# luanfujun/Langevin-MCMC

Measured on AMD Instinct MI355X. Metric: MALA chain-steps/sec, torus scene, higher is better.
Workload: dtype f32

## Files before the change

include/lmc_abi.h:

```cpp
#ifndef LMC_ABI_H
#define LMC_ABI_H

#ifdef __cplusplus
extern "C" {
#endif

typedef struct lmc_ctx lmc_ctx;

typedef struct lmc_scene_desc {
    const char *scene_xml;
    int force_diffuse;
    int max_depth;
    int width, height;
    int seed_offset;
    int device;
    int use_gradient;
} lmc_scene_desc;

const char *lmc_last_error(void);

lmc_ctx *lmc_create(const lmc_scene_desc *desc);
void lmc_destroy(lmc_ctx *ctx);
int lmc_device_count(void);

// ... 35 lines not shown
int lmc_mc_stats(lmc_ctx *ctx, long long *out2);
int lmc_mc_accumulate(lmc_ctx *ctx, int spp, long long stream_begin, long long stream_end);
int lmc_mc_coverage(lmc_ctx *ctx, long long *ranges, int cap);
int lmc_mc_read_fixed(lmc_ctx *ctx, long long *words);
int lmc_mc_overflow(lmc_ctx *ctx, long long *n);
int lmc_group_mc_render(lmc_ctx **ctxs, int n, int spp, long long stream_begin, long long stream_end);
int lmc_group_mc_accumulate(lmc_ctx **ctxs, int n, int spp, long long stream_begin, long long stream_end);
int lmc_mc_save(lmc_ctx *ctx, const char *path);
int lmc_mc_load(lmc_ctx *ctx, const char *path);
long long lmc_mc_file_info(const char *path, char *json, long long cap);
int lmc_mc_layer_info(lmc_ctx *ctx, int *mode, int *n_layers, int *cl, int cap);
int lmc_mc_read_layer(lmc_ctx *ctx, int layer, float *rgb);
int lmc_mc_read_layer_fixed(lmc_ctx *ctx, int layer, long long *words);
int lmc_mc_coverage_probe(const long long *adds, int n_adds, long long total, int *accepted, long long *cov, int cov_cap, int *n_cov, long long *comp, int comp_cap, int *n_comp);
int lmc_mc_chunks_probe(long long begin, long long end, long long n_tiles, long long launch_streams, long long *out, int cap);
int lmc_stats(lmc_ctx *ctx, long long *out8, double *weight_sum);
int lmc_chain_summary(lmc_ctx *ctx, int which, float *out, int stride);
int lmc_relocation_stats(lmc_ctx *ctx, long long *out4);
long long lmc_relocation_skipped(lmc_ctx *ctx);
int lmc_resident_stats(lmc_ctx *ctx, long long *out4, double *kernel_ms);
int lmc_step_timing(lmc_ctx *ctx, double *kernel_ms, long long *launches);
int lmc_kernel_timing(lmc_ctx *ctx, double *out3);
int lmc_kernel_timing_split(lmc_ctx *ctx, double *out4);

int lmc_comm_unique_id(unsigned char *out128);
int lmc_comm_init(lmc_ctx *ctx, int n_ranks, int rank, const unsigned char *id128);
int lmc_film_allreduce(lmc_ctx *ctx);
#define LMC_COMM_MAX_SCALARS 64
int lmc_comm_allreduce_f64(lmc_ctx *ctx, double *vals, int n, int op);
int lmc_comm_barrier(lmc_ctx *ctx);
void *lmc_film_device_ptr(lmc_ctx *ctx, long long *n_floats);

int lmc_grad_batch(int c, int l, int n, const float *primary_soa, const float *scene38, const float *vert_soa, float *loglum, float *grad_soa);

int lmc_hess_batch(int c, int l, int n, const float *primary_soa, const float *scene38, const float *vert_soa, float *loglum, float *grad_soa, float *hess_soa);

int lmc_cache_rows(lmc_ctx *ctx, int dim, float *pss, float *weight, float *extra);
int lmc_cache_probe(lmc_ctx *ctx, int dim, int n, const float *u, int *row, const float *query, const int *cl, float *pdf);

int lmc_trace(lmc_ctx *ctx, int n, const float *rays, int *prim, float *t);
int lmc_occluded(lmc_ctx *ctx, int n, const float *rays, int *occluded);
int lmc_rng_probe(int n_seeds, const unsigned long long *seeds, int mode, int n, float mean, float stddev, unsigned *out);
int lmc_kd_probe(int dim, int npts, const float *pts, int nq, const float *q, float radius_sq, int knn, int *out_n, int *out_idx, float *out_dist);
int lmc_lower_bound_probe(int n, const float *cdf, int nq, const float *u, int *out);
int lmc_layout_probe(int nChains, int words, int mode, int batch, int reps, double *msPerLaunch);
int lmc_lean_plan_probe(int bvh_stack_need, int block_threads, int *stack_words, int *lds_words_per_thread, long long *lds_bytes_per_block);
// ... 66 lines not shown
```

langevin-mcmc_amd/__init__.py:

```python
import ctypes
import os

import numpy as np

_HERE = os.path.dirname(os.path.abspath(__file__))
ROOT = os.path.dirname(_HERE)
LIB_PATH = os.environ.get("LMC_LIB") or os.path.join(_HERE, "liblmc_hip.so")
vp = ctypes.c_void_p
c_ll = ctypes.c_longlong


class SceneDesc(ctypes.Structure):
    _fields_ = [
        ("scene_xml", ctypes.c_char_p),
        ("force_diffuse", ctypes.c_int),
        ("max_depth", ctypes.c_int),
        ("width", ctypes.c_int),
        ("height", ctypes.c_int),
        ("seed_offset", ctypes.c_int),
        ("device", ctypes.c_int),
        ("use_gradient", ctypes.c_int),
    ]


# ... 14 lines not shown
        L.lmc_create.restype = vp
        L.lmc_create.argtypes = [ctypes.POINTER(SceneDesc)]
        L.lmc_destroy.argtypes = [vp]
        L.lmc_info.argtypes = [vp, vp]
        L.lmc_scene_params.argtypes = [vp, vp]
        L.lmc_set_option.argtypes = [vp, ctypes.c_char_p, ctypes.c_double]
        L.lmc_chains_init.argtypes = [vp, c_ll, ctypes.c_int, ctypes.c_int, ctypes.c_int, ctypes.c_int, c_ll, c_ll]
        L.lmc_init_result.argtypes = [vp, vp, vp]
        L.lmc_chains_step.argtypes = [vp, ctypes.c_int]
        L.lmc_sync.argtypes = [vp]
        L.lmc_film_read.argtypes = [vp, vp]
        L.lmc_film_clear.argtypes = [vp]
        L.lmc_stats.argtypes = [vp, vp, vp]
        L.lmc_chain_summary.argtypes = [vp, ctypes.c_int, vp, ctypes.c_int]
        L.lmc_step_timing.argtypes = [vp, vp, vp]
        L.lmc_relocation_stats.argtypes = [vp, vp]
        if hasattr(L, "lmc_resident_stats"):
            L.lmc_resident_stats.argtypes = [vp, vp, vp]
        if hasattr(L, "lmc_relocation_skipped"):
            L.lmc_relocation_skipped.argtypes = [vp]
            L.lmc_relocation_skipped.restype = c_ll
        L.lmc_kernel_timing.argtypes = [vp, vp]
        L.lmc_kernel_timing_split.argtypes = [vp, vp]
        L.lmc_get_option.argtypes = [vp, ctypes.c_char_p, vp]
        L.lmc_output_name.argtypes = [vp]
        L.lmc_output_name.restype = ctypes.c_char_p
        L.lmc_image_read.argtypes = [ctypes.c_char_p, vp, vp, vp]
        L.lmc_image_write_exr.argtypes = [ctypes.c_char_p, vp, ctypes.c_int, ctypes.c_int]
        L.lmc_direct_lighting.argtypes = [vp, ctypes.c_int]
        L.lmc_direct_read.argtypes = [vp, vp]
        L.lmc_path_trace.argtypes = [vp, ctypes.c_int]
        L.lmc_bidir_mc.argtypes = [vp, ctypes.c_int]
        if hasattr(L, "lmc_mc_render"):
            L.lmc_mc_render.argtypes = [vp, ctypes.c_int, c_ll, c_ll]
            L.lmc_mc_read.argtypes = [vp, vp]
            L.lmc_mc_stats.argtypes = [vp, vp]
        if hasattr(L, "lmc_mc_accumulate"):
            L.lmc_mc_accumulate.argtypes = [vp, ctypes.c_int, c_ll, c_ll]
            L.lmc_mc_coverage.argtypes = [vp, vp, ctypes.c_int]
            L.lmc_mc_read_fixed.argtypes = [vp, vp]
            L.lmc_mc_overflow.argtypes = [vp, vp]
            L.lmc_group_mc_render.argtypes = [vp, ctypes.c_int, ctypes.c_int, c_ll, c_ll]
            L.lmc_group_mc_accumulate.argtypes = [vp, ctypes.c_int, ctypes.c_int, c_ll, c_ll]
            L.lmc_mc_save.argtypes = [vp, ctypes.c_char_p]
            L.lmc_mc_load.argtypes = [vp, ctypes.c_char_p]
            L.lmc_mc_file_info.argtypes = [ctypes.c_char_p, ctypes.c_char_p, c_ll]
# ... 367 lines not shown
        if lib().lmc_step_table(self.h, P(out), 1 if clear else 0) != 0:
            raise RuntimeError(_err())
        return out

    def step_timing(self):
        ms = ctypes.c_double()
        n = c_ll()
        if lib().lmc_step_timing(self.h, ctypes.byref(ms), ctypes.byref(n)) != 0:
            raise RuntimeError(_err())
        return ms.value, n.value

    def kernel_timing(self):
        out = (ctypes.c_double * 3)()
        if lib().lmc_kernel_timing(self.h, out) != 0:
            raise RuntimeError(_err())
        return out[0], out[1], int(out[2])

    def kernel_timing_split(self):
        out = (ctypes.c_double * 4)()
        if lib().lmc_kernel_timing_split(self.h, out) != 0:
            raise RuntimeError(_err())
        return {"lean_ms": out[0], "large_ms": out[1], "generic_ms": out[2], "lean_steps": int(out[3])}

    def lean_info(self):
        out = (ctypes.c_int * 16)()
        L = lib()
        L.lmc_lean_info.argtypes = [vp, ctypes.POINTER(ctypes.c_int)]
        if L.lmc_lean_info(self.h, out) != 0:
            raise RuntimeError(_err())
        v = list(out)
        return dict(leaf_hist=v[:8], stack_need=v[8], stack_words=v[9], lds=v[10], glossy=v[11], lightless=v[12], quant=v[13], tight=v[14], block=v[15])

    def trace(self, rays):
        rays = np.ascontiguousarray(rays, np.float32)
        n = len(rays)
        prim = np.zeros(n, np.int32)
        t = np.zeros(n, np.float32)
        if lib().lmc_trace(self.h, n, P(rays), P(prim), P(t)) != 0:
            raise RuntimeError(_err())
        return prim, t

    def occluded(self, rays):
        rays = np.ascontiguousarray(rays, np.float32)
        occ = np.zeros(len(rays), np.int32)
        if lib().lmc_occluded(self.h, len(rays), P(rays), P(occ)) != 0:
            raise RuntimeError(_err())
# ... 381 lines not shown
```

langevin-mcmc_amd/csrc/device/kernels.h:

```cpp
#pragma once
#include <hip/hip_runtime.h>

#include "dchain.h"
#include "dstep_params.h"

namespace lmcd {
struct H2Arrays;
struct MalaPipe;
struct H2Bins;
struct H2MCParam;
}

void LaunchSeedRng(int n, long long firstSeed, uint64_t *state, uint32_t *tab, hipStream_t s);
void LaunchLowerBoundProbe(int n, const float *cdf, int nq, const float *u, int *out, hipStream_t s);
void LaunchRngProbe(int nSeeds, const unsigned long long *seeds, int mode, int n, float mean, float stddev, uint32_t *tabScratch, uint32_t *out, hipStream_t s);
void LaunchPluginGrad(int c, int l, const float *in, float *out, int wantGrad, hipStream_t s);
void LaunchPluginHess(int c, int l, const float *in, float *stage , float *out, hipStream_t s);
void LaunchCacheProbe(const lmcd::DCache *cache, int dim, int n, const float *u, int *row, const float *query, const int *cl, float *pdf, hipStream_t s);
void LaunchTransProbe(int n, int mode, const float *x, const float *y, float *o, hipStream_t s);
void LaunchShadeProbe(const lmcd::DScene &S, int op, bool glossy, int n, const int *ints, const float *in, int *ok, float *out, hipStream_t s);
void LaunchStreamProbe(long long nWords, const float *in, float *out, hipStream_t s);
void LaunchAddInto(float *dst, const float *src, size_t n, hipStream_t s);
void LaunchAddIntoF64(double *dst, const double *src, size_t n, hipStream_t s);
void LaunchAddIntoI64(long long *dst, const long long *src, size_t n, hipStream_t s);
// ... 77 lines not shown
                   const int *listCount, int bvhStackNeed, bool glossy, int gridBlocks, hipStream_t s);
void LaunchMalaFinish(const lmcd::DScene &S, const lmcd::DCache *cache, const lmcd::ChainArrays &A, const lmcd::Film &film, const lmcd::StepParams &P, const lmcd::MalaPipe &M,
                      const int *list, const int *listCount, int gridBlocks, hipStream_t s);
void LaunchMalaGrad(const float *rec, const lmcd::H2Bins &bins, int N, const float *scene38 , float *gout, int gridBlocks, hipStream_t s);
void LaunchHessBatch(int c, int l, int n, const float *primarySoA, const float *scene, const float *vertSoA, float *logLum, float *gradSoA, float *hessSoA,
                     hipStream_t s);
void LaunchBuildLists(const lmcd::ChainArrays &A, const lmcd::NextLists &next, int sortPlain, unsigned leanDims, hipStream_t s);
void LaunchInitLists(int n, int *large, int *counts, hipStream_t s);
void LaunchCachePush(const lmcd::ChainArrays &A, const lmcd::CachePushTargets &T, unsigned long long *tileCounts, int *stageCounts , hipStream_t s);
void LaunchCachePushApply(const float *gathered, size_t stageFloats, int world, const lmcd::PushStageLayout &lay, const lmcd::CachePushTargets &T,
                          int *hostCounts , hipStream_t s);
void LaunchLayoutProbe(int N, int words, int mode, int batch, const float *in, float *out, hipStream_t s);
void LaunchSortByTechnique(const unsigned char *nextKind, const int *in, int *out, const int *count, int *blockHist, int maxEntries, hipStream_t s);
void LaunchInclusiveScan(int *v, int n, int *tileSums, hipStream_t s);
struct RelocBuffers {
    unsigned *placedKey;
    int *tileCount, *tileHist;
    int *members;
    int *sorted;
    int *count;
    float *staging;
    int capacity;
    bool fine;
};
size_t RelocTiles(int N);
size_t RelocRecordWords(int maxDepth);
void LaunchRelocIota(int n, int *v, hipStream_t s);
void LaunchRelocate(const lmcd::ChainArrays &A, int maxDepth, const RelocBuffers &B, bool withoutGaussianOnly, hipStream_t s);
void LaunchRelocPlan(const lmcd::ChainArrays &A, int maxDepth, const RelocBuffers &B, bool withoutGaussianOnly, hipStream_t s);
void LaunchRelocFineKey(const lmcd::ChainArrays &A, const int *leafPosOfTri, int numTris, int mode, unsigned long long *keys, const lmcd::TriData *tris, const lmcd::DMaterial *materials, hipStream_t s);
void LaunchRelocMove(const lmcd::ChainArrays &A, int maxDepth, const RelocBuffers &B, hipStream_t s, int keyMode = 0);
struct RelocSortBuffers {
    unsigned *keys[2];
    int *vals[2];
    int *hist;
    int *scanSums;
};
size_t RelocSortBlocks(int N);
void LaunchRadixSort24(const RelocSortBuffers &W, const int *nPtr, int nMax, int *out, hipStream_t s);
void LaunchRelocFullSort(const lmcd::ChainArrays &A, int maxDepth, const RelocBuffers &B, const RelocSortBuffers &W, hipStream_t s);
void LaunchRelocateFine(const lmcd::ChainArrays &A, int maxDepth, const RelocBuffers &B, const RelocSortBuffers &W, bool withoutGaussianOnly, hipStream_t s);
void LaunchBuildCacheGrid(const float *pts, int n, int dim, int G, int m, const int *coord, int *scratchStart, int *scratchCursor, int *scratchWordCount, int *tileSums,
                          uint2 *words, int *cellStart, unsigned short *idx, hipStream_t s);
size_t CkptRecordWords(int maxDepth, bool sampleCache, bool h2mc);
void LaunchCkptPack(const lmcd::ChainArrays &A, int maxDepth, bool sampleCache, const float *h2Gauss, int first, int n, float *staging, hipStream_t s);
void LaunchCkptUnpack(const lmcd::ChainArrays &A, int maxDepth, bool sampleCache, float *h2Gauss, int first, int n, const float *staging, hipStream_t s);
void LaunchLatchKind(const lmcd::ChainArrays &A, const int *large, const int *generic, const int *lean, const int *counts, unsigned char *kindOf, hipStream_t s);
void LaunchChainRows(const lmcd::ChainArrays &A, int which, const int *ids, int n, const unsigned char *kindOf, float *out, hipStream_t s);
// ... 2 lines not shown
```

langevin-mcmc_amd/csrc/device/relocate.hip:

```cpp
#include "dstep.h"
#include "kernels.h"

namespace lmcd {
namespace {

enum : int { RW_FLAGS = 0, RW_SAMPLEIDX, RW_NUMSAMPLES, RW_ADJREJECT, RW_SPLATCOUNT, RW_CHAINID, RW_SCORESUM, RW_LASTSCORESUM, RW_LASTSCORE, RW_PATHWEIGHT, RW_NEXTKIND, RW_RNG_LO, RW_RNG_HI, RW_KEY, RW_RNG_TICKED, RW_SCALARS = 16 };
constexpr int RW_TAB = RW_SCALARS, RW_HEAD = RW_TAB + 64, RW_VERT = RW_HEAD + DPATH_HEAD_WORDS;

struct RecordLayout {
    int nV, nS;
    LMC_HD int Contrib() const { return RW_VERT + 2 * nV * DVERTEX_WORDS; }
    LMC_HD int Splats() const { return Contrib() + CONTRIB_WORDS; }
    LMC_HD int Vectors() const { return Splats() + nS * SPLAT_WORDS; }
    LMC_HD int Gauss() const { return Vectors() + 7 * MAXPSS; }
    LMC_HD int Words() const { return Gauss() + GAUSS_WORDS; }
};

#ifndef LMC_RELOC_ORDER
#define LMC_RELOC_ORDER 1
#endif
#ifndef LMC_RELOC_TILES
#define LMC_RELOC_TILES 0
#endif
LMC_D int SlotKey(const ChainArrays &A, int i, int tiles) {
// ... 31 lines not shown
constexpr int RELOC_TILE = 1024;
LMC_D int MemberKey(const ChainArrays &A, const unsigned *placedKey, int i, bool withoutGaussianOnly, int tiles) {
    if (i >= A.N || A.stepKind[i] != NEXT_LARGE) return -1;
    const int key = SlotKey(A, i, tiles);
    if ((unsigned)key == placedKey[i]) return -1;
    if (withoutGaussianOnly && (A.flags[i] & F_GAUSS)) return -1;
    return key;
}
__global__ void __launch_bounds__(64) k_reloc_count(ChainArrays A, const unsigned *placedKey, int *tileCount, int *tileHist, bool noGauss, int tiles) {
    __shared__ int h[64];
    h[threadIdx.x] = 0;
    __syncthreads();
    const int base = blockIdx.x * RELOC_TILE + threadIdx.x;
    int total = 0;
    for (int j = 0; j < RELOC_TILE / 64; j++) {
        const int key = MemberKey(A, placedKey, base + 64 * j, noGauss, tiles);
        if (key >= 0) atomicAdd(&h[key], 1), total++;
    }
    __syncthreads();
    tileHist[blockIdx.x * 64 + threadIdx.x] = h[threadIdx.x];
    for (int off = 32; off > 0; off >>= 1) total += __shfl_down(total, off);
    if (threadIdx.x == 0) tileCount[blockIdx.x] = total;
}
__global__ void __launch_bounds__(64) k_reloc_offsets(int nTiles, int *tileCount, int *tileHist, int *count, int capacity) {
    const int key = threadIdx.x;
    int total = 0;
#pragma unroll 8
    for (int t = 0; t < nTiles; t++) total += tileHist[t * 64 + key];
    int incl = total;
    for (int off = 1; off < 64; off <<= 1) {
        const int o = __shfl_up(incl, off);
        if (key >= off) incl += o;
    }
    if (key == 63) {
        if (incl > capacity) count[0] = 0, count[1]++;
        else
            count[0] = incl;
    }
    int run = incl - total;
#pragma unroll 8
    for (int t = 0; t < nTiles; t++) {
        const int c = tileHist[t * 64 + key];
        tileHist[t * 64 + key] = run;
        run += c;
    }
    int carry = 0;
    for (int b = 0; b < nTiles; b += 64) {
        const int t = b + threadIdx.x, v = t < nTiles ? tileCount[t] : 0;
        int in = v;
        for (int off = 1; off < 64; off <<= 1) {
            const int o = __shfl_up(in, off);
            if (key >= off) in += o;
        }
        if (t < nTiles) tileCount[t] = carry + in - v;
        carry += __shfl(in, 63);
    }
}
__global__ void __launch_bounds__(64) k_reloc_assign(ChainArrays A, const unsigned *placedKey, const int *tileStart, const int *groupStart, int *members, int *sorted, bool noGauss, int tiles) {
    __shared__ int cursor[64];
    cursor[threadIdx.x] = groupStart[blockIdx.x * 64 + threadIdx.x];
    __syncthreads();
    const int base = blockIdx.x * RELOC_TILE + threadIdx.x;
    int m0 = tileStart[blockIdx.x];
    for (int j = 0; j < RELOC_TILE / 64; j++) {
        const int key = MemberKey(A, placedKey, base + 64 * j, noGauss, tiles);
        const unsigned long long mask = __ballot(key >= 0);
        const unsigned long long below = (1ull << threadIdx.x) - 1ull;
        if (key >= 0) members[m0 + __popcll(mask & below)] = base + 64 * j;
        unsigned long long todo = mask;
        while (todo) {
            const int k = __shfl(key, __ffsll((long long)todo) - 1);
            const unsigned long long same = __ballot(key == k);
            if (key == k) sorted[cursor[k] + __popcll(same & below)] = m0 + __popcll(mask & below);
            __syncthreads();
            if (threadIdx.x == 0) cursor[k] += __popcll(same);
            __syncthreads();
            todo &= ~same;
        }
        m0 += __popcll(mask);
    }
}

LMC_D float *VectorBase(const ChainArrays &A, int v) {
    float *const b[7] = {A.chV1, A.chV2, A.chCurrNewV2, A.chPropNewV1, A.chPropNewV2, A.chPss, A.chLastPss};
    return b[v];
}
// ... 422 lines not shown
        m0 += __popcll(mask);
    }
}

__global__ void __launch_bounds__(256) k_reloc_iota(int n, int *v) {
    const int i = blockIdx.x * 256 + threadIdx.x;
    if (i < n) v[i] = i;
}

}
}

using namespace lmcd;

static RecordLayout MakeRecordLayout(int maxDepth) {
    RecordLayout R;
    R.nV = std::min(MAXD, std::max(maxDepth, 1));
    R.nS = std::min(MAXCONTRIB, (maxDepth + 1) * (maxDepth + 2) / 2);
    return R;
}
size_t RelocRecordWords(int maxDepth) { return (size_t)MakeRecordLayout(maxDepth).Words(); }
void LaunchRelocIota(int n, int *v, hipStream_t s) { hipLaunchKernelGGL(k_reloc_iota, dim3((n + 255) / 256), dim3(256), 0, s, n, v); }
size_t RelocTiles(int N) { return (size_t)(N + RELOC_TILE - 1) / RELOC_TILE; }

static void LaunchMoveKernels(const ChainArrays &A, const RecordLayout &R, const RelocBuffers &B, int tiles, int moveBlocks, hipStream_t s) {
    static const bool coop = !(getenv("LMC_RELOC_COOP") && atoi(getenv("LMC_RELOC_COOP")) == 0);
    if (coop) {
        hipLaunchKernelGGL(k_reloc_gather_coop, dim3(moveBlocks), dim3(64), 0, s, A, R, B.members, B.count, B.staging, B.capacity, tiles);
        hipLaunchKernelGGL(k_reloc_scatter_coop, dim3(moveBlocks), dim3(64), 0, s, A, R, B.members, B.sorted, B.count, B.staging, B.placedKey, B.capacity);
    } else {
        hipLaunchKernelGGL(k_reloc_gather, dim3(moveBlocks), dim3(64), 0, s, A, R, B.members, B.sorted, B.count, B.staging, B.capacity, tiles);
        hipLaunchKernelGGL(k_reloc_scatter, dim3(moveBlocks), dim3(64), 0, s, A, R, B.members, B.sorted, B.count, B.staging, B.placedKey, B.capacity);
    }
}
void LaunchRelocFineKey(const ChainArrays &A, const int *leafPosOfTri, int numTris, int mode, unsigned long long *keys, const TriData *tris, const DMaterial *materials, hipStream_t s) {
    hipLaunchKernelGGL(k_reloc_finekey, dim3((A.N + 255) / 256), dim3(256), 0, s, A, leafPosOfTri, numTris, mode, keys, tris, materials);
}
void LaunchRelocMove(const ChainArrays &A, int maxDepth, const RelocBuffers &B, hipStream_t s, int keyMode) {
    const RecordLayout R = MakeRecordLayout(maxDepth);
    const int moveBlocks = std::min((A.N + 63) / 64, 65536);
    LaunchMoveKernels(A, R, B, keyMode, moveBlocks, s);
}

size_t RelocSortBlocks(int N) { return (size_t)(N + RS_TILE - 1) / RS_TILE; }
void LaunchRadixSort24(const RelocSortBuffers &W, const int *nPtr, int nMax, int *out, hipStream_t s) {
    const int nBlocks = (int)RelocSortBlocks(nMax);
// ... 7 lines not shown
        hipLaunchKernelGGL(k_rs_scatter, dim3(nBlocks), dim3(64), 0, s, kin[pass], vin[pass], kout[pass], vout[pass], nPtr, nMax, 8 * pass, W.hist, nBlocks);
    }
}
void LaunchRelocFullSort(const ChainArrays &A, int maxDepth, const RelocBuffers &B, const RelocSortBuffers &W, hipStream_t s) {
    const int N = A.N;
    hipLaunchKernelGGL(k_rs_set_count, dim3(1), dim3(64), 0, s, B.count, N);
    hipLaunchKernelGGL(k_rs_key, dim3((N + 255) / 256), dim3(256), 0, s, A, W.keys[0]);
    LaunchRadixSort24(W, B.count, N, B.sorted, s);
    hipLaunchKernelGGL(k_reloc_iota, dim3((N + 255) / 256), dim3(256), 0, s, N, B.members);
    LaunchRelocMove(A, maxDepth, B, s, B.fine ? -1 : 0);
}
void LaunchRelocateFine(const ChainArrays &A, int maxDepth, const RelocBuffers &B, const RelocSortBuffers &W, bool withoutGaussianOnly, hipStream_t s) {
    const RecordLayout R = MakeRecordLayout(maxDepth);
    const int N = A.N, nTiles = (N + RELOC_TILE - 1) / RELOC_TILE;
    hipLaunchKernelGGL(k_relf_count, dim3(nTiles), dim3(64), 0, s, A, B.placedKey, B.tileCount, withoutGaussianOnly);
    hipLaunchKernelGGL(k_relf_offsets, dim3(1), dim3(64), 0, s, nTiles, B.tileCount, B.count, B.capacity);
    hipLaunchKernelGGL(k_relf_assign, dim3(nTiles), dim3(64), 0, s, A, B.placedKey, B.tileCount, B.count, B.members, W.keys[0], withoutGaussianOnly);
    LaunchRadixSort24(W, B.count, B.capacity, B.sorted, s);
    const int moveBlocks = std::min((N + 63) / 64, 4096);
    LaunchMoveKernels(A, R, B, -1, moveBlocks, s);
}

void LaunchRelocPlan(const ChainArrays &A, int maxDepth, const RelocBuffers &B, bool withoutGaussianOnly, hipStream_t s) {
    const int N = A.N, nTiles = (N + RELOC_TILE - 1) / RELOC_TILE;
    const int tiles = (LMC_RELOC_TILES && maxDepth <= 6) ? 8 : 0;
    hipLaunchKernelGGL(k_reloc_count, dim3(nTiles), dim3(64), 0, s, A, B.placedKey, B.tileCount, B.tileHist, withoutGaussianOnly, tiles);
    hipLaunchKernelGGL(k_reloc_offsets, dim3(1), dim3(64), 0, s, nTiles, B.tileCount, B.tileHist, B.count, B.capacity);
    hipLaunchKernelGGL(k_reloc_assign, dim3(nTiles), dim3(64), 0, s, A, B.placedKey, B.tileCount, B.tileHist, B.members, B.sorted, withoutGaussianOnly, tiles);
}
void LaunchRelocate(const ChainArrays &A, int maxDepth, const RelocBuffers &B, bool withoutGaussianOnly, hipStream_t s) {
    const RecordLayout R = MakeRecordLayout(maxDepth);
    const int N = A.N;
    const int tiles = (LMC_RELOC_TILES && maxDepth <= 6) ? 8 : 0;
    LaunchRelocPlan(A, maxDepth, B, withoutGaussianOnly, s);
    const int moveBlocks = std::min((N + 63) / 64, 4096);
    LaunchMoveKernels(A, R, B, tiles, moveBlocks, s);
}
```

langevin-mcmc_amd/csrc/host/context.cpp:

```cpp
#include <hip/hip_runtime.h>
#include <dlfcn.h>

#include <algorithm>
#include <chrono>
#include <condition_variable>
#include <mutex>
#include <cstdio>
#include <cstdlib>
#include <cstring>
#include <exception>
#include <functional>
#include <memory>
#include <stdexcept>
#include <string>
#include <thread>
#include <vector>

#include <rccl/rccl.h>

#include "../../../include/lmc_abi.h"
#include "../device/drng.h"
#include "../device/kernels.h"
#include "../device/upload.h"
#include "../device/dh2coop.h"
// ... 771 lines not shown
    else
        c->chPath.Free(), c->chContrib.Free();
    c->pathWeight.Alloc(N), c->lastScoreSum.Alloc(N), c->lastScore.Alloc(N), c->contribList.Alloc(N * MAXCONTRIB * CONTRIB_WORDS, false);
    c->pushData.Alloc(N * GAUSS_WORDS), c->flags.Alloc(N), c->nextKind.Alloc(N + 4), c->adjacentReject.Alloc(N), c->sampleIdx.Alloc(N), c->numSamples.Alloc(N), c->pushDim.Alloc(N);
    c->counters.Alloc(8), c->weightSum.Alloc(1), c->prof.Alloc(16);
    ChainArrays &A = c->A;
    A.N = (int)N;
    A.rngState = c->rngState.p, A.rngTab = c->rngTab.p, A.rngTicked = c->rngTicked.p, A.curPath = c->curPath.p, A.pathBuf1 = c->pathBuf1.p, A.curContrib = c->curContrib.p, A.scoreSum = c->scoreSum.p;
    A.flags = c->flags.p, A.gaussian = c->gaussian.p, A.gaussian1 = c->gaussian1.p, A.curSplat = c->curSplat.p, A.curSplatCount = c->curSplatCount.p;
    A.chV1 = c->chV1.p, A.chV2 = c->chV2.p, A.chCurrNewV2 = c->chCurrNewV2.p, A.chPropNewV1 = c->chPropNewV1.p, A.chPropNewV2 = c->chPropNewV2.p,
    A.chPss = c->chPss.p, A.chLastPss = c->chLastPss.p;
    A.chPath = sampleCache ? c->chPath.p : nullptr, A.chContrib = sampleCache ? c->chContrib.p : nullptr;
    A.pathWeight = c->pathWeight.p, A.lastScoreSum = c->lastScoreSum.p, A.lastScore = c->lastScore.p;
    A.adjacentReject = c->adjacentReject.p, A.sampleIdx = c->sampleIdx.p, A.numSamples = c->numSamples.p;
    A.contribList = c->contribList.p, A.nextKind = c->nextKind.p, A.pushDim = c->pushDim.p, A.pushData = c->pushData.p;
    A.initPath = c->initPath.p, A.initContrib = c->initContrib.p, A.initScoreSum = c->initScoreSum.p, A.initLsAll = c->initLsAll.p, A.initCLAll = c->initCLAll.p;
    A.counters = c->counters.p, A.weightSum = c->weightSum.p, A.prof = c->prof.p;
    c->relocate = true;
    if (const char *e = getenv("LMC_RELOCATE")) c->relocate = atoi(e) != 0;
    if (sampleCache) c->relocate = false;
    c->relocations = 0;
    if (c->relocate) {
        c->chainId.Alloc(N, false), c->slotOf.Alloc(N, false), c->relocTileCount.Alloc(RelocTiles((int)N) + 1, false), c->relocTileHist.Alloc(RelocTiles((int)N) * 64, false), c->relocMembers.Alloc(N, false);
        c->relocSorted.Alloc(N, false), c->relocCount.Alloc(2), c->relocPlacedKey.Alloc(N, false), c->stepKind.Alloc(N + 4, false);
        c->relocStaging.Alloc(N * RelocRecordWords(c->S.opt.maxDepth), false);
        HIP_CHECK(hipMemsetAsync(c->relocPlacedKey.p, 0xff, N * sizeof(unsigned), s));
        HIP_CHECK(hipMemsetAsync(c->stepKind.p, NEXT_LARGE, N, s));
        LaunchRelocIota((int)N, c->chainId.p, s), LaunchRelocIota((int)N, c->slotOf.p, s);
        c->resortEvery = 32;
        if (const char *e = getenv("LMC_RESORT_EVERY")) c->resortEvery = std::max(0, atoi(e));
        if (c->resortEveryOpt >= 0) c->resortEvery = c->resortEveryOpt;
        c->resortFirst = 4;
        if (const char *e = getenv("LMC_RESORT_FIRST")) c->resortFirst = std::max(0, atoi(e));
        if (c->resortFirstOpt >= 0) c->resortFirst = c->resortFirstOpt;
        if (c->S.opt.h2mc) c->resortEvery = 0;
        c->stepsSinceInit = 0, c->resorts = 0;
        c->relocFine = false;
        if (const char *e = getenv("LMC_RELOC_FINE")) c->relocFine = atoi(e) != 0;
        if (c->resortEvery > 0 || c->relocFine) {
            const size_t nb = RelocSortBlocks((int)N);
            for (int k = 0; k < 2; k++) c->sortKeys[k].Alloc(N, false), c->sortVals[k].Alloc(N, false);
            c->sortHist.Alloc(256 * nb, false), c->sortScanSums.Alloc(256 * nb / 2048 + 2, false);
            c->RS = RelocSortBuffers{{c->sortKeys[0].p, c->sortKeys[1].p}, {c->sortVals[0].p, c->sortVals[1].p}, c->sortHist.p, c->sortScanSums.p};
        }
        c->RB = RelocBuffers{c->relocPlacedKey.p, c->relocTileCount.p, c->relocTileHist.p, c->relocMembers.p, c->relocSorted.p, c->relocCount.p, c->relocStaging.p, (int)N, c->relocFine};
        A.chainId = c->chainId.p, A.slotOf = c->slotOf.p, A.stepKind = c->stepKind.p;
    } else {
        A.chainId = nullptr, A.slotOf = nullptr, A.stepKind = nullptr;
        for (auto *b : {&c->chainId, &c->slotOf, &c->relocTileCount, &c->relocTileHist, &c->relocMembers, &c->relocSorted, &c->relocCount}) b->Free();
        c->relocPlacedKey.Free(), c->stepKind.Free(), c->relocStaging.Free();
    }
    if (!U.fromCheckpoint) {
        LaunchSeedRng((int)N, (long long)chainBegin + c->S.opt.seedOffset, c->rngState.p, c->rngTab.p, s);
        LaunchSetupChains(A, chainBegin, perChain, chainsNeedExtra, s);
    }
    c->stepGrid = (int)std::min<size_t>((N + 255) / 256, 4096);
    c->gradStride = c->stepGrid * 256;
    if (const char *e = getenv("LMC_LEAN_BLOCK")) c->leanBlock = std::max(64, std::min(256, atoi(e) / 64 * 64));
    c->sortPlain = c->S.glossy ? 4 : 0;
    if (const char *e = getenv("LMC_SORT_PLAIN")) c->sortPlain = atoi(e);
    c->gradBuf.Alloc(c->useGradient ? (size_t)c->gradStride * 640 : 1, false);
    size_t maxGridCells = 0;
    for (int d = 0; d <= PSS_MAX_LENGTH; d++) {
        CacheDimHost &cd = c->cacheDims[d];
        cd.ready = false;
        cd.relevant = (d % 2 == 0) && d >= 2 * std::max(c->S.opt.minDepth, 3) && d <= 2 * c->S.opt.maxDepth;
        if (cd.relevant) {
            cd.pss.Alloc((size_t)PSS_MAX_SIZE * d), cd.v1.Alloc((size_t)PSS_MAX_SIZE * d), cd.v2.Alloc((size_t)PSS_MAX_SIZE * d);
            cd.weight.Alloc(PSS_MAX_SIZE);
            if (sampleCache) cd.extra.Alloc((size_t)PSS_MAX_SIZE * CACHE_ROW_EXTRA), cd.distCdf.Alloc(PSS_MAX_SIZE + 1);
            cd.gridG = CacheGridG(d), cd.gridM = std::min(c->gridDims, d);
            size_t cells = 1, nbrs = 1;
// ... 550 lines not shown
            CachePack(c, sL);
            if (c->world == 1 && c->earlyApply) CacheApplyLaunch(c, sL), c->appliedEarly = true;
            else if (c->world > 1 && c->group.size() <= 1 && c->comm && c->earlyApply && RcclEarlyExchange() && c->stageLayout.totalFloats > 0) {
                RcclCheck(GetRccl().AllGather(c->pushStage.p, c->pushGather.p, (size_t)c->stageLayout.totalFloats * sizeof(float), ncclUint8, (ncclComm_t)c->comm, sL),
                          "ncclAllGather(cache pushes, large-step stream)");
                CacheApplyLaunch(c, sL), c->appliedEarly = true;
            }
        }
        if (c->relocate) {
            if (c->relocations == 2 && c->RB.capacity == (int)c->N && c->N >= 65536 && c->resortEvery == 0 && !getenv("LMC_RELOC_STAGING_FULL")) {
                static std::mutex stagingMutex;
                std::lock_guard<std::mutex> lock(stagingMutex);
                HIP_CHECK(hipStreamSynchronize(sL));
                const size_t cap = c->N / 2;
                c->RB.staging = nullptr, c->RB.capacity = 0;
                c->relocStaging.Alloc(cap * RelocRecordWords(c->S.opt.maxDepth), false);
                c->RB.staging = c->relocStaging.p, c->RB.capacity = (int)cap;
            }
            if (c->relocFine) LaunchRelocateFine(c->A, c->S.opt.maxDepth, c->RB, c->RS, c->S.opt.h2mc != 0, sL);
            else
                LaunchRelocate(c->A, c->S.opt.maxDepth, c->RB, c->S.opt.h2mc != 0, sL);
            c->relocations++;
        }
    };
    if (!genericFirst) large();
    if (c->timing) HIP_CHECK(hipEventRecord(ev.e[6], sG));
    LaunchGeneric(c, film, P, cur, cnt, next, sG);
    if (c->timing) HIP_CHECK(hipEventRecord(ev.e[7], sG));
    if (genericFirst) large();
    if (c->timing) HIP_CHECK(hipEventRecord(ev.e[1], s));
    if (!c->S.opt.h2mc) LaunchStepSmallPlain(c->S, c->cacheDev.p, c->A, film, P, c->lists[cur][2].p, cnt + 2, next, c->bvhDepth, c->S.glossy != 0, c->leanLdsStack, c->leanBlock, c->profileLean, s);
    if (c->timing) HIP_CHECK(hipEventRecord(ev.e[2], s));
    if (c->overlap) {
        HIP_CHECK(hipEventRecord(c->joinEvent[0], sL));
        HIP_CHECK(hipStreamWaitEvent(s, c->joinEvent[0], 0));
        if (c->needGeneric) {
            HIP_CHECK(hipEventRecord(c->joinEvent[1], sG));
            HIP_CHECK(hipStreamWaitEvent(s, c->joinEvent[1], 0));
        }
    }
    return exchange;
}
void DebugResort(lmc_ctx *c) {
    hipStream_t s = c->stream;
    const int mode = c->pendingResort;
    c->pendingResort = 0;
// ... 231 lines not shown
int lmc_group_chains_step(lmc_ctx **ctxs, int n, int nSteps) {
    LMC_TRY
    std::vector<lmc_ctx *> g(ctxs, ctxs + n);
    for (lmc_ctx *c : g)
        if (c->group != g) throw std::runtime_error("lmc_group_chains_step: not the group lmc_group_chains_init set up");
    RunSteps(g, nSteps);
    return 0;
    LMC_CATCH(-1)
}

int lmc_sync(lmc_ctx *c) {
    LMC_TRY
    HIP_CHECK(hipSetDevice(c->device));
    HIP_CHECK(hipStreamSynchronize(c->stream));
    return 0;
    LMC_CATCH(-1)
}

int lmc_step_timing(lmc_ctx *c, double *kernelMs, long long *launches) {
    LMC_TRY
    HIP_CHECK(hipStreamSynchronize(c->stream));
    double ms = 0;
    c->smallMs = c->largeMs = c->largeOnlyMs = c->genericMs = 0;
    for (auto &ev : c->events) {
        float t = 0;
        HIP_CHECK(hipEventElapsedTime(&t, ev.e[0], ev.e[3]));
        ms += t;
        HIP_CHECK(hipEventElapsedTime(&t, ev.e[1], ev.e[2]));
        c->smallMs += t;
        HIP_CHECK(hipEventElapsedTime(&t, ev.e[4], ev.e[5]));
        c->largeMs += t, c->largeOnlyMs += t;
        HIP_CHECK(hipEventElapsedTime(&t, ev.e[6], ev.e[7]));
        c->largeMs += t, c->genericMs += t;
        c->eventPool.push_back(ev);
    }
    if (kernelMs) *kernelMs = ms;
    if (launches) *launches = (long long)c->events.size();
    c->events.clear();
    return 0;
    LMC_CATCH(-1)
}

int lmc_kernel_timing(lmc_ctx *c, double *out3) {
    LMC_TRY
    HIP_CHECK(hipStreamSynchronize(c->stream));
    out3[0] = c->smallMs, out3[1] = c->largeMs;
    out3[2] = (double)c->counters.Download()[7];
    return 0;
    LMC_CATCH(-1)
}

int lmc_kernel_timing_split(lmc_ctx *c, double *out4) {
    LMC_TRY
    HIP_CHECK(hipStreamSynchronize(c->stream));
    out4[0] = c->smallMs, out4[1] = c->largeOnlyMs, out4[2] = c->genericMs;
    out4[3] = (double)c->counters.Download()[7];
    return 0;
    LMC_CATCH(-1)
}

int lmc_prof_read(lmc_ctx *c, unsigned long long *out16) {
    LMC_TRY
    HIP_CHECK(hipSetDevice(c->device));
    HIP_CHECK(hipStreamSynchronize(c->stream));
    if (c->prof.n == 0) throw std::runtime_error("lmc_prof_read before lmc_chains_init");
    std::vector<unsigned long long> h = c->prof.Download();
    for (int k = 0; k < 16; k++) out16[k] = h[k];
    HIP_CHECK(hipMemset(c->prof.p, 0, 16 * sizeof(unsigned long long)));
    return 0;
    LMC_CATCH(-1)
}

int lmc_group_film_reduce(lmc_ctx **ctxs, int n, double *out_ms) {
    LMC_TRY
    std::vector<lmc_ctx *> g(ctxs, ctxs + n);
    for (lmc_ctx *c : g) {
        if (c->group != g) throw std::runtime_error("lmc_group_film_reduce: not the group lmc_group_chains_init set up");
        if (c->filmReduced) throw std::runtime_error("lmc_group_film_reduce: the films already hold the sum over the members; step or clear them first");
        if (c->film.n != g[0]->film.n) throw std::runtime_error("lmc_group_film_reduce: the members' films differ in size");
// ... 307 lines not shown
```

langevin-mcmc_amd/csrc/host/context.h:

```cpp
#pragma once
#include <chrono>
#include <memory>
#include <string>
#include <utility>
#include <vector>

#include "../../../include/lmc_abi.h"
#include "../device/kernels.h"
#include "../device/dh2coop.h"
#include "accel.h"
#include "hostutil.h"
#include "mcfilm.h"
#include "scene.h"

using namespace lmcd;
using namespace lmc_host;

namespace lmc_host {

struct CacheDimHost {
    DevBuf<float> pss, v1, v2, weight;
    DevBuf<float> extra, distCdf;
    DevBuf<KdNode> nodes;
    DevBuf<uint2> gridWords;
// ... 93 lines not shown
    DevBuf<unsigned char> rngTicked;
    DevBuf<float> curPath, pathBuf1, curContrib, scoreSum, gaussian, gaussian1, curSplat, chV1, chV2, chCurrNewV2, chPropNewV1, chPropNewV2, chPss, chLastPss, chPath, chContrib, pathWeight,
        lastScoreSum, lastScore, contribList, pushData, initPath, initContrib, initScoreSum, initLsAll;
    DevBuf<unsigned char> initCLAll;
    DevBuf<unsigned char> nextKind;
    DevBuf<int> flags, curSplatCount, adjacentReject, sampleIdx, numSamples, pushDim;
    DevBuf<unsigned long long> counters, prof;
    bool profileLean = false;
    DevBuf<double> weightSum;
    DevBuf<float> gradBuf;
    DevBuf<float> h2Rec, h2Out, h2Gauss, h2Offset, h2Py, h2Px, h2PropContrib;
    DevBuf<int> h2Step, h2Items, h2BinOf, h2Counts, h2SubList, h2SubCount;
    H2Bins h2Bins[H2_MAX_PARTS][2] = {};
    int h2Parts = 1, h2PartStride = 0;
    const int *h2SplitOf = nullptr;
    DevBuf<unsigned char> h2Kind;
    H2Arrays H2{};
    int h2HessGrid = 0, h2GaussGrid = 0;
    bool malaPipe = true;
    MalaPipe MP{};
    int gradStride = 0, stepGrid = 0;
    int leanBlock = 64, sortPlain = 0;
    bool relocate = false;
    DevBuf<int> chainId, slotOf, relocTileCount, relocTileHist, relocMembers, relocSorted, relocCount;
    DevBuf<unsigned> relocPlacedKey;
    DevBuf<unsigned char> stepKind;
    bool relocFine = false;
    DevBuf<float> relocStaging;
    RelocBuffers RB{};
    long long relocations = 0;
    int pendingResort = 0;
    int resortEvery = 0, resortFirst = 0;
    int resortEveryOpt = -1, resortFirstOpt = -1;
    long long stepsSinceInit = 0, resorts = 0;
    DevBuf<unsigned> sortKeys[2];
    DevBuf<int> sortVals[2], sortHist, sortScanSums;
    RelocSortBuffers RS{};
    DevBuf<int> lists[2][3], listCounts[2];
    int parity = 0;
    CacheDimHost cacheDims[PSS_MAX_LENGTH + 1];
    DCache cacheHost;
    DevBuf<DCache> cacheDev;
    DevBuf<int> cacheCounts;
    DevBuf<unsigned long long> pushTiles;
    DevBuf<int> gridScratchStart, gridScratchCursor, gridScratchWordCount, gridTileSums;
    CachePushTargets pushT;
    CachePushTargets stageT;
// ... 12 lines not shown
    bool rowsPrefetched[CACHE_SLOTS] = {false, false, false, false};
    int lastDelta[CACHE_SLOTS] = {0, 0, 0, 0};
    char *treePinned[CACHE_SLOTS] = {nullptr, nullptr, nullptr, nullptr};
    hipEvent_t treesUpEvent = nullptr;
    bool allCachesReady = false;
    int residentSteps = 0, residentLanes = 0;
    long long residentLaunches = 0, lockSteps = 0;
    double residentMs = 0;
    std::vector<std::pair<hipEvent_t, hipEvent_t>> residentEvents;
    DevBuf<unsigned long long> residentGuard;
    bool residentResortPending = false;
    int mutationAtInit = -1;
    lmc_host::ChainDiag *diag = nullptr;
    bool needGeneric = true;
    bool genericTokenOnly = false;
    float normalization = 0.f;
    std::vector<float> lengthFunc, lengthCdf;
    float lengthFuncInt = 0.f;
    long long numInitContribs = 0;
    std::vector<unsigned char> initCL;
    std::vector<float> initLs;
    std::vector<unsigned long long> initOffsets;
    struct StepEvents {
        hipEvent_t e[8];
    };
    bool timing = false;
    std::vector<StepEvents> events, eventPool;
    double smallMs = 0, largeMs = 0, largeOnlyMs = 0, genericMs = 0;
    ~lmc_ctx() {
        for (lmc_ctx *peer : group)
            if (peer != this) {
                peer->group.clear();
                peer->world = 1, peer->rank = 0;
            }
        for (auto *v : {&events, &eventPool})
            for (auto &ev : *v)
                for (auto e : ev.e) (void)hipEventDestroy(e);
        if (comm) {
            try {
                (void)GetRcclDestroy(comm);
            } catch (...) {
            }
        }
        if (hostCounts) (void)hipHostFree(hostCounts);
        for (float *r : rowsPinned)
            if (r) (void)hipHostFree(r);
        for (char *r : treePinned)
            if (r) (void)hipHostFree(r);
        if (treesUpEvent) (void)hipEventDestroy(treesUpEvent);
        if (cachePinned) (void)hipHostFree(cachePinned);
        for (auto e : h2HeadDone)
// ... 52 lines not shown
```

langevin-mcmc_amd/csrc/host/list_probes.cpp:

```cpp
#include <hip/hip_runtime.h>

#include <algorithm>
#include <cstdint>
#include <cstring>
#include <stdexcept>
#include <string>
#include <vector>

#include "../../../include/lmc_abi.h"
#include "../device/kernels.h"
#include "../device/dh2coop.h"
#include "../device/dh2mc.h"
#include "hostutil.h"

using namespace lmcd;

static_assert(LMC_PROBE_BINS == H2_NBINS, "include/lmc_abi.h: LMC_PROBE_BINS is the number of bins of a pipeline stage");
static_assert(LMC_PROBE_CACHE_ROWS == PSS_MAX_SIZE, "include/lmc_abi.h: LMC_PROBE_CACHE_ROWS is the row count of a cache dim");
static_assert(PSS_MAX_LENGTH == 12 && CACHE_SLOTS == 4, "lmc_cache_push_probe lays its rows out for the dims 6, 8, 10, 12");

namespace {

template <class T>
struct Buf {
// ... 211 lines not shown
        const int dim = 6 + 2 * sl;
        for (int a = 0; a < 3; a++) {
            const std::vector<float> r = rows[sl][a].Download();
            for (int row = 0; row < PSS_MAX_SIZE; row++)
                memcpy(out_rows + ((size_t)(sl * 3 + a) * PSS_MAX_SIZE + row) * PSS_MAX_LENGTH, r.data() + (size_t)row * dim, (size_t)dim * sizeof(float));
        }
        weight[sl].Download(out_weights + (size_t)sl * PSS_MAX_SIZE, PSS_MAX_SIZE);
    }
    dCount.Download(out_counts, CACHE_SLOTS), dDim.Download(out_push_dim, N);
    return 0;
    LMC_CATCH(-1)
}

int lmc_reloc_plan_probe(int N, const unsigned char *step_kind, const int *c, const int *l, const int *flags, const unsigned *placed_key, int without_gaussian_only,
                         int capacity, int skipped_before, int *out_count, int *out_members, int *out_sorted) {
    LMC_TRY
    Require(N >= 1 && step_kind && c && l && flags && placed_key && capacity >= 0 && out_count && out_members && out_sorted, "lmc_reloc_plan_probe: bad arguments");
    std::vector<float> contrib((size_t)2 * N);
    memcpy(contrib.data(), c, (size_t)N * 4), memcpy(contrib.data() + N, l, (size_t)N * 4);
    const int count0[2] = {kSentinel, skipped_before};
    Stream st;
    Buf<unsigned char> sk;
    Buf<float> con;
    Buf<int> fl, tileCount, tileHist, members, sorted, count;
    Buf<unsigned> placed;
    sk.Upload(step_kind, N), con.Upload(contrib), fl.Upload(flags, N), placed.Upload(placed_key, N);
    tileCount.Fill(RelocTiles(N) + 1, kSentinel), tileHist.Fill(RelocTiles(N) * 64, kSentinel);
    members.Fill(N, kSentinel), sorted.Fill(N, kSentinel), count.Upload(count0, 2);
    ChainArrays A;
    memset(&A, 0, sizeof(A));
    A.N = N, A.stepKind = sk.p, A.curContrib = con.p, A.flags = fl.p;
    const RelocBuffers B{placed.p, tileCount.p, tileHist.p, members.p, sorted.p, count.p, nullptr, capacity, false};
    LaunchRelocPlan(A, 6, B, without_gaussian_only != 0, st.s);
    st.Finish();
    count.Download(out_count, 2), members.Download(out_members, N), sorted.Download(out_sorted, N);
    return 0;
    LMC_CATCH(-1)
}

}

namespace {

float Untouched() {
    const uint32_t bits = 0x7fc0beefu;
    float f;
    memcpy(&f, &bits, 4);
    return f;
}

template <class Fits>
void RequireWorkList(const std::string &who, int N, int n_list, const int *items, const int *count, const int *start, int grid_blocks, Fits fits, const char *techArg) {
    auto fail = [&](const std::string &what) { throw std::runtime_error(who + ": " + what); };
    if (n_list < 1) fail("n_list = " + std::to_string(n_list) + ": a list needs at least one entry (n = 0 is not a call)");
    if (N < n_list) fail("N = " + std::to_string(N) + " is smaller than n_list = " + std::to_string(n_list));
// ... 127 lines not shown
```

Before: 799.1 million.

## Replace single-block relocation offset scan with two-level super-tile prefix sums

```diff
diff --git a/include/lmc_abi.h b/include/lmc_abi.h
--- a/include/lmc_abi.h
+++ b/include/lmc_abi.h
@@ -81,6 +81,7 @@
 int lmc_step_timing(lmc_ctx *ctx, double *kernel_ms, long long *launches);
 int lmc_kernel_timing(lmc_ctx *ctx, double *out3);
 int lmc_kernel_timing_split(lmc_ctx *ctx, double *out4);
+int lmc_step_path_timing(lmc_ctx *ctx, double *out4);
 
 int lmc_comm_unique_id(unsigned char *out128);
 int lmc_comm_init(lmc_ctx *ctx, int n_ranks, int rank, const unsigned char *id128);
diff --git a/langevin-mcmc_amd/__init__.py b/langevin-mcmc_amd/__init__.py
--- a/langevin-mcmc_amd/__init__.py
+++ b/langevin-mcmc_amd/__init__.py
@@ -60,6 +60,8 @@
             L.lmc_relocation_skipped.restype = c_ll
         L.lmc_kernel_timing.argtypes = [vp, vp]
         L.lmc_kernel_timing_split.argtypes = [vp, vp]
+        if hasattr(L, "lmc_step_path_timing"):
+            L.lmc_step_path_timing.argtypes = [vp, vp]
         L.lmc_get_option.argtypes = [vp, ctypes.c_char_p, vp]
         L.lmc_output_name.argtypes = [vp]
         L.lmc_output_name.restype = ctypes.c_char_p
@@ -473,6 +475,12 @@
             raise RuntimeError(_err())
         return {"lean_ms": out[0], "large_ms": out[1], "generic_ms": out[2], "lean_steps": int(out[3])}
 
+    def step_path_timing(self):
+        out = (ctypes.c_double * 4)()
+        if lib().lmc_step_path_timing(self.h, out) != 0:
+            raise RuntimeError(_err())
+        return {"lean_end_ms": out[0], "large_end_ms": out[1], "side_end_ms": out[2], "step_end_ms": out[3]}
+
     def lean_info(self):
         out = (ctypes.c_int * 16)()
         L = lib()
diff --git a/langevin-mcmc_amd/csrc/device/kernels.h b/langevin-mcmc_amd/csrc/device/kernels.h
--- a/langevin-mcmc_amd/csrc/device/kernels.h
+++ b/langevin-mcmc_amd/csrc/device/kernels.h
@@ -123,8 +123,10 @@
     float *staging;
     int capacity;
     bool fine;
+    int *superCount, *superHist;
 };
 size_t RelocTiles(int N);
+size_t RelocSuperTiles(int N);
 size_t RelocRecordWords(int maxDepth);
 void LaunchRelocIota(int n, int *v, hipStream_t s);
 void LaunchRelocate(const lmcd::ChainArrays &A, int maxDepth, const RelocBuffers &B, bool withoutGaussianOnly, hipStream_t s);
diff --git a/langevin-mcmc_amd/csrc/device/relocate.hip b/langevin-mcmc_amd/csrc/device/relocate.hip
--- a/langevin-mcmc_amd/csrc/device/relocate.hip
+++ b/langevin-mcmc_amd/csrc/device/relocate.hip
@@ -77,46 +77,53 @@
     for (int off = 32; off > 0; off >>= 1) total += __shfl_down(total, off);
     if (threadIdx.x == 0) tileCount[blockIdx.x] = total;
 }
-__global__ void __launch_bounds__(64) k_reloc_offsets(int nTiles, int *tileCount, int *tileHist, int *count, int capacity) {
-    const int key = threadIdx.x;
-    int total = 0;
-#pragma unroll 8
-    for (int t = 0; t < nTiles; t++) total += tileHist[t * 64 + key];
+constexpr int RELOC_SUPER = 64;
+LMC_D int SumRows(const int *rows, int n) {
+    int sum = 0;
+    for (int r0 = 0; r0 < n; r0 += 16) {
+        int v[16];
+#pragma unroll
+        for (int r = 0; r < 16; r++) v[r] = rows[min(r0 + r, n - 1) * 64 + threadIdx.x];
+#pragma unroll
+        for (int r = 0; r < 16; r++) sum += r0 + r < n ? v[r] : 0;
+    }
+    return sum;
+}
+__global__ void __launch_bounds__(64) k_reloc_super(int nTiles, const int *tileCount, const int *tileHist, int *superCount, int *superHist) {
+    const int t0 = blockIdx.x * RELOC_SUPER, nt = min(RELOC_SUPER, nTiles - t0);
+    superHist[blockIdx.x * 64 + threadIdx.x] = SumRows(tileHist + (size_t)t0 * 64, nt);
+    int total = (int)threadIdx.x < nt ? tileCount[t0 + threadIdx.x] : 0;
+    for (int off = 32; off > 0; off >>= 1) total += __shfl_down(total, off);
+    if (threadIdx.x == 0) superCount[blockIdx.x] = total;
+}
+__global__ void __launch_bounds__(64) k_reloc_assign(ChainArrays A, const unsigned *placedKey, int nSuper, const int *tileCount, const int *tileHist, const int *superCount, const int *superHist,
+                                                     int *members, int *sorted, int *count, int capacity, bool noGauss, int tiles) {
+    __shared__ int cursor[64];
+    const int key = threadIdx.x, super = blockIdx.x / RELOC_SUPER, inSuper = blockIdx.x % RELOC_SUPER, t0 = super * RELOC_SUPER;
+    int before = SumRows(tileHist + (size_t)t0 * 64, inSuper), total = 0;
+    for (int s0 = 0; s0 < nSuper; s0 += RELOC_SUPER) {
+        const int n = min(RELOC_SUPER, nSuper - s0), nFront = min(max(super - s0, 0), n);
+        const int front = SumRows(superHist + (size_t)s0 * 64, nFront);
+        before += front;
+        total += front + SumRows(superHist + (size_t)(s0 + nFront) * 64, n - nFront);
+    }
+    int first = key < inSuper ? tileCount[t0 + key] : 0;
+    for (int s = key; s < super; s += 64) first += superCount[s];
     int incl = total;
     for (int off = 1; off < 64; off <<= 1) {
         const int o = __shfl_up(incl, off);
         if (key >= off) incl += o;
     }
-    if (key == 63) {
+    for (int off = 32; off > 0; off >>= 1) first += __shfl_xor(first, off);
+    if (blockIdx.x == 0 && key == 63) {
         if (incl > capacity) count[0] = 0, count[1]++;
         else
             count[0] = incl;
     }
-    int run = incl - total;
-#pragma unroll 8
-    for (int t = 0; t < nTiles; t++) {
-        const int c = tileHist[t * 64 + key];
-        tileHist[t * 64 + key] = run;
-        run += c;
-    }
-    int carry = 0;
-    for (int b = 0; b < nTiles; b += 64) {
-        const int t = b + threadIdx.x, v = t < nTiles ? tileCount[t] : 0;
-        int in = v;
-        for (int off = 1; off < 64; off <<= 1) {
-            const int o = __shfl_up(in, off);
-            if (key >= off) in += o;
-        }
-        if (t < nTiles) tileCount[t] = carry + in - v;
-        carry += __shfl(in, 63);
-    }
-}
-__global__ void __launch_bounds__(64) k_reloc_assign(ChainArrays A, const unsigned *placedKey, const int *tileStart, const int *groupStart, int *members, int *sorted, bool noGauss, int tiles) {
-    __shared__ int cursor[64];
-    cursor[threadIdx.x] = groupStart[blockIdx.x * 64 + threadIdx.x];
+    cursor[key] = incl - total + before;
     __syncthreads();
     const int base = blockIdx.x * RELOC_TILE + threadIdx.x;
-    int m0 = tileStart[blockIdx.x];
+    int m0 = first;
     for (int j = 0; j < RELOC_TILE / 64; j++) {
         const int key = MemberKey(A, placedKey, base + 64 * j, noGauss, tiles);
         const unsigned long long mask = __ballot(key >= 0);
@@ -585,6 +592,7 @@
 size_t RelocRecordWords(int maxDepth) { return (size_t)MakeRecordLayout(maxDepth).Words(); }
 void LaunchRelocIota(int n, int *v, hipStream_t s) { hipLaunchKernelGGL(k_reloc_iota, dim3((n + 255) / 256), dim3(256), 0, s, n, v); }
 size_t RelocTiles(int N) { return (size_t)(N + RELOC_TILE - 1) / RELOC_TILE; }
+size_t RelocSuperTiles(int N) { return (RelocTiles(N) + RELOC_SUPER - 1) / RELOC_SUPER; }
 
 static void LaunchMoveKernels(const ChainArrays &A, const RecordLayout &R, const RelocBuffers &B, int tiles, int moveBlocks, hipStream_t s) {
     static const bool coop = !(getenv("LMC_RELOC_COOP") && atoi(getenv("LMC_RELOC_COOP")) == 0);
@@ -638,11 +646,12 @@
 }
 
 void LaunchRelocPlan(const ChainArrays &A, int maxDepth, const RelocBuffers &B, bool withoutGaussianOnly, hipStream_t s) {
-    const int N = A.N, nTiles = (N + RELOC_TILE - 1) / RELOC_TILE;
+    const int N = A.N, nTiles = (N + RELOC_TILE - 1) / RELOC_TILE, nSuper = (nTiles + RELOC_SUPER - 1) / RELOC_SUPER;
     const int tiles = (LMC_RELOC_TILES && maxDepth <= 6) ? 8 : 0;
     hipLaunchKernelGGL(k_reloc_count, dim3(nTiles), dim3(64), 0, s, A, B.placedKey, B.tileCount, B.tileHist, withoutGaussianOnly, tiles);
-    hipLaunchKernelGGL(k_reloc_offsets, dim3(1), dim3(64), 0, s, nTiles, B.tileCount, B.tileHist, B.count, B.capacity);
-    hipLaunchKernelGGL(k_reloc_assign, dim3(nTiles), dim3(64), 0, s, A, B.placedKey, B.tileCount, B.tileHist, B.members, B.sorted, withoutGaussianOnly, tiles);
+    hipLaunchKernelGGL(k_reloc_super, dim3(nSuper), dim3(64), 0, s, nTiles, B.tileCount, B.tileHist, B.superCount, B.superHist);
+    hipLaunchKernelGGL(k_reloc_assign, dim3(nTiles), dim3(64), 0, s, A, B.placedKey, nSuper, B.tileCount, B.tileHist, B.superCount, B.superHist, B.members, B.sorted, B.count, B.capacity,
+                       withoutGaussianOnly, tiles);
 }
 void LaunchRelocate(const ChainArrays &A, int maxDepth, const RelocBuffers &B, bool withoutGaussianOnly, hipStream_t s) {
     const RecordLayout R = MakeRecordLayout(maxDepth);
diff --git a/langevin-mcmc_amd/csrc/host/context.cpp b/langevin-mcmc_amd/csrc/host/context.cpp
--- a/langevin-mcmc_amd/csrc/host/context.cpp
+++ b/langevin-mcmc_amd/csrc/host/context.cpp
@@ -817,6 +817,7 @@
     c->relocations = 0;
     if (c->relocate) {
         c->chainId.Alloc(N, false), c->slotOf.Alloc(N, false), c->relocTileCount.Alloc(RelocTiles((int)N) + 1, false), c->relocTileHist.Alloc(RelocTiles((int)N) * 64, false), c->relocMembers.Alloc(N, false);
+        c->relocSuperCount.Alloc(RelocSuperTiles((int)N), false), c->relocSuperHist.Alloc(RelocSuperTiles((int)N) * 64, false);
         c->relocSorted.Alloc(N, false), c->relocCount.Alloc(2), c->relocPlacedKey.Alloc(N, false), c->stepKind.Alloc(N + 4, false);
         c->relocStaging.Alloc(N * RelocRecordWords(c->S.opt.maxDepth), false);
         HIP_CHECK(hipMemsetAsync(c->relocPlacedKey.p, 0xff, N * sizeof(unsigned), s));
@@ -838,11 +839,11 @@
             c->sortHist.Alloc(256 * nb, false), c->sortScanSums.Alloc(256 * nb / 2048 + 2, false);
             c->RS = RelocSortBuffers{{c->sortKeys[0].p, c->sortKeys[1].p}, {c->sortVals[0].p, c->sortVals[1].p}, c->sortHist.p, c->sortScanSums.p};
         }
-        c->RB = RelocBuffers{c->relocPlacedKey.p, c->relocTileCount.p, c->relocTileHist.p, c->relocMembers.p, c->relocSorted.p, c->relocCount.p, c->relocStaging.p, (int)N, c->relocFine};
+        c->RB = RelocBuffers{c->relocPlacedKey.p, c->relocTileCount.p, c->relocTileHist.p, c->relocMembers.p, c->relocSorted.p, c->relocCount.p, c->relocStaging.p, (int)N, c->relocFine, c->relocSuperCount.p, c->relocSuperHist.p};
         A.chainId = c->chainId.p, A.slotOf = c->slotOf.p, A.stepKind = c->stepKind.p;
     } else {
         A.chainId = nullptr, A.slotOf = nullptr, A.stepKind = nullptr;
-        for (auto *b : {&c->chainId, &c->slotOf, &c->relocTileCount, &c->relocTileHist, &c->relocMembers, &c->relocSorted, &c->relocCount}) b->Free();
+        for (auto *b : {&c->chainId, &c->slotOf, &c->relocTileCount, &c->relocTileHist, &c->relocSuperCount, &c->relocSuperHist, &c->relocMembers, &c->relocSorted, &c->relocCount}) b->Free();
         c->relocPlacedKey.Free(), c->stepKind.Free(), c->relocStaging.Free();
     }
     if (!U.fromCheckpoint) {
@@ -1439,6 +1440,7 @@
                 LaunchRelocate(c->A, c->S.opt.maxDepth, c->RB, c->S.opt.h2mc != 0, sL);
             c->relocations++;
         }
+        if (c->timing) HIP_CHECK(hipEventRecord(ev.e[8], sL));
     };
     if (!genericFirst) large();
     if (c->timing) HIP_CHECK(hipEventRecord(ev.e[6], sG));
@@ -1716,10 +1718,16 @@
     HIP_CHECK(hipStreamSynchronize(c->stream));
     double ms = 0;
     c->smallMs = c->largeMs = c->largeOnlyMs = c->genericMs = 0;
+    for (double &p : c->pathMs) p = 0;
     for (auto &ev : c->events) {
         float t = 0;
         HIP_CHECK(hipEventElapsedTime(&t, ev.e[0], ev.e[3]));
-        ms += t;
+        ms += t, c->pathMs[3] += t;
+        const int pathEnd[3] = {2, 5, 8};
+        for (int k = 0; k < 3; k++) {
+            HIP_CHECK(hipEventElapsedTime(&t, ev.e[0], ev.e[pathEnd[k]]));
+            c->pathMs[k] += t;
+        }
         HIP_CHECK(hipEventElapsedTime(&t, ev.e[1], ev.e[2]));
         c->smallMs += t;
         HIP_CHECK(hipEventElapsedTime(&t, ev.e[4], ev.e[5]));
@@ -1749,6 +1757,14 @@
     HIP_CHECK(hipStreamSynchronize(c->stream));
     out4[0] = c->smallMs, out4[1] = c->largeOnlyMs, out4[2] = c->genericMs;
     out4[3] = (double)c->counters.Download()[7];
+    return 0;
+    LMC_CATCH(-1)
+}
+
+int lmc_step_path_timing(lmc_ctx *c, double *out4) {
+    LMC_TRY
+    HIP_CHECK(hipStreamSynchronize(c->stream));
+    for (int k = 0; k < 4; k++) out4[k] = c->pathMs[k];
     return 0;
     LMC_CATCH(-1)
 }
diff --git a/langevin-mcmc_amd/csrc/host/context.h b/langevin-mcmc_amd/csrc/host/context.h
--- a/langevin-mcmc_amd/csrc/host/context.h
+++ b/langevin-mcmc_amd/csrc/host/context.h
@@ -139,7 +139,7 @@
     int gradStride = 0, stepGrid = 0;
     int leanBlock = 64, sortPlain = 0;
     bool relocate = false;
-    DevBuf<int> chainId, slotOf, relocTileCount, relocTileHist, relocMembers, relocSorted, relocCount;
+    DevBuf<int> chainId, slotOf, relocTileCount, relocTileHist, relocSuperCount, relocSuperHist, relocMembers, relocSorted, relocCount;
     DevBuf<unsigned> relocPlacedKey;
     DevBuf<unsigned char> stepKind;
     bool relocFine = false;
@@ -198,11 +198,12 @@
     std::vector<float> initLs;
     std::vector<unsigned long long> initOffsets;
     struct StepEvents {
-        hipEvent_t e[8];
+        hipEvent_t e[9];
     };
     bool timing = false;
     std::vector<StepEvents> events, eventPool;
     double smallMs = 0, largeMs = 0, largeOnlyMs = 0, genericMs = 0;
+    double pathMs[4] = {0, 0, 0, 0};
     ~lmc_ctx() {
         for (lmc_ctx *peer : group)
             if (peer != this) {
diff --git a/langevin-mcmc_amd/csrc/host/list_probes.cpp b/langevin-mcmc_amd/csrc/host/list_probes.cpp
--- a/langevin-mcmc_amd/csrc/host/list_probes.cpp
+++ b/langevin-mcmc_amd/csrc/host/list_probes.cpp
@@ -257,15 +257,16 @@
     Stream st;
     Buf<unsigned char> sk;
     Buf<float> con;
-    Buf<int> fl, tileCount, tileHist, members, sorted, count;
+    Buf<int> fl, tileCount, tileHist, superCount, superHist, members, sorted, count;
     Buf<unsigned> placed;
     sk.Upload(step_kind, N), con.Upload(contrib), fl.Upload(flags, N), placed.Upload(placed_key, N);
     tileCount.Fill(RelocTiles(N) + 1, kSentinel), tileHist.Fill(RelocTiles(N) * 64, kSentinel);
+    superCount.Fill(RelocSuperTiles(N), kSentinel), superHist.Fill(RelocSuperTiles(N) * 64, kSentinel);
     members.Fill(N, kSentinel), sorted.Fill(N, kSentinel), count.Upload(count0, 2);
     ChainArrays A;
     memset(&A, 0, sizeof(A));
     A.N = N, A.stepKind = sk.p, A.curContrib = con.p, A.flags = fl.p;
-    const RelocBuffers B{placed.p, tileCount.p, tileHist.p, members.p, sorted.p, count.p, nullptr, capacity, false};
+    const RelocBuffers B{placed.p, tileCount.p, tileHist.p, members.p, sorted.p, count.p, nullptr, capacity, false, superCount.p, superHist.p};
     LaunchRelocPlan(A, 6, B, without_gaussian_only != 0, st.s);
     st.Finish();
     count.Download(out_count, 2), members.Download(out_members, N), sorted.Download(out_sorted, N);
```

Result: no change. 797.5 million (-0.2%).
